# GuanRunwei/Achelous

Hardware: AMD Instinct MI355X
Metric: frames/sec (whole node) EN-GDF-PN-S0 320x320+512pts bs64 @1/2/4/8 GPU (higher is better)
Workload: dtype bf16; 1 GPU; EN-GDF-PN-S0 forward + decode + NMS, 320x320 image + radar map, 512 points, batch 64 per GPU, all 5 heads, seeded random weights; radar_map=256 occupied cells per frame of 102 400 (SURVEY 8d: real maps are > 99 % zeros), global_batch=64, parallelism=batch-sharded x1, launches_per_forward=113

## Files before the change

### achelous_amd/csrc/api.cpp

```cpp
#include <atomic>
#include <cstring>
#include <functional>
#include <string>

#include "engine.h"
#include <map>
#include <mutex>
#include <algorithm>
#include "k_detect.h"
#include "k_prepost.h"
#include "k_train.h"
#include "k_train2.h"
#include "k_train3.h"
#include "k_loss.h"
#include "k_metrics.h"

struct ach_handle {
    ach::EngineBase* eng = nullptr;
    std::string err;
};

static thread_local std::string g_create_error;

template <class F>
// ... 9 lines not shown
        h->err = e.what();
        return ACH_ERR_INVALID;
    } catch (...) {
        h->err = "unknown error";
        return ACH_ERR_INVALID;
    }
}

extern "C" {

int ach_create(const ach_config* cfg, ach_handle** out) {
    if (!cfg || !out) return ACH_ERR_INVALID;
    try {
        if (cfg->backbone != ACH_BACKBONE_EDGENEXT && cfg->backbone != ACH_BACKBONE_MOBILEVIT)
            throw ach::AchError{ACH_ERR_UNSUPPORTED, "backbone must be 'en' or 'mv'"};
        if (cfg->phi < ACH_PHI_S0 || cfg->phi > ACH_PHI_S2) throw ach::AchError{ACH_ERR_UNSUPPORTED, "phi must be S0, S1 or S2"};
        if (cfg->neck != ACH_NECK_GDF && cfg->neck != ACH_NECK_CDF) throw ach::AchError{ACH_ERR_UNSUPPORTED, "neck must be 'gdf' or 'cdf'"};
        if (cfg->pc_seg != ACH_PCSEG_PN && cfg->pc_seg != ACH_PCSEG_PN2 && cfg->pc_seg != ACH_PCSEG_NONE && cfg->pc_seg != ACH_PCSEG_PN2_MSG)
            throw ach::AchError{ACH_ERR_UNSUPPORTED, "pc_seg must be 'pn', 'pn2', 'pn2_msg' or none (Achelous3T)"};
        if (cfg->num_det < 1 || cfg->num_det > 59 || cfg->num_seg < 1 || (cfg->pc_seg != ACH_PCSEG_NONE && (cfg->pc_classes < 1 || cfg->pc_channels < 3)))
            throw ach::AchError{ACH_ERR_INVALID, "bad class / channel counts"};
        ach_handle* h = new ach_handle();
        h->eng = ach::make_engine(*cfg);
        *out = h;
        return ACH_OK;
    } catch (const ach::AchError& e) {
        g_create_error = e.msg;
        return e.code;
    } catch (...) {
        g_create_error = "allocation failure";
        return ACH_ERR_NOMEM;
    }
}

void ach_destroy(ach_handle* h) {
    if (!h) return;
    delete h->eng;
    delete h;
}

const char* ach_last_error(const ach_handle* h) { return h ? h->err.c_str() : g_create_error.c_str(); }

int ach_load_weights(ach_handle* h, const ach_tensor_desc* tensors, size_t n) {
    return guarded(h, [&] { h->eng->load(tensors, n); });
}

int ach_set_option(ach_handle* h, const char* key, int32_t value) {
    return guarded(h, [&] {
        if (!key) throw ach::AchError{ACH_ERR_INVALID, "null option"};
        if (std::string(key) == "full_taps") h->eng->full_taps = value != 0;
        else if (std::string(key) == "streams") h->eng->multi_stream = value != 0;
        else if (std::string(key) == "graph") h->eng->use_graph = value != 0;
        else if (std::string(key) == "fused_mlp") h->eng->fuse_mlp = value != 0;
        else if (std::string(key) == "mlp_split") h->eng->mlp_split = value;
        else if (std::string(key) == "row_conv") h->eng->row_conv = value != 0;
        else if (std::string(key) == "fused_rc") h->eng->fuse_rc = value != 0;
        else if (std::string(key) == "dw_tile") h->eng->dw_tile = value != 0;
        else if (std::string(key) == "stem_mfma") h->eng->stem_mfma = value != 0;
        else if (std::string(key) == "point_stream2") h->eng->point_on_head_stream = value;
        else if (std::string(key) == "head_batch") h->eng->head_batch = value != 0;
        else if (std::string(key) == "head_fuse") h->eng->head_fuse = value != 0;
        else if (std::string(key) == "head_fuse_dbg") h->eng->head_fuse_dbg = value;
        else if (std::string(key) == "side_priority") h->eng->side_low_priority = value;
        else if (std::string(key) == "head_lds_pad") h->eng->head_lds_pad = value < 0 ? 0 : (value > 65536 ? 65536 : value);
        else if (std::string(key) == "head_stream") h->eng->head_stream = value != 0;
        else if (std::string(key) == "split_decoders") h->eng->split_decoders = value;
        else if (std::string(key) == "group_wpc") h->eng->group_wpc = value < 0 ? 0 : value;
        else if (std::string(key) == "group_max") h->eng->group_max = value < 0 ? 0 : value;
        else if (std::string(key) == "dec_fork") h->eng->dec_fork = value < 0 ? 0 : (value > 3 ? 3 : value);
        else if (std::string(key) == "radar_start") h->eng->radar_start = value;
        else if (std::string(key) == "pipeline") h->eng->pipeline = value != 0;
        else if (std::string(key) == "pool_strip") h->eng->pool_strip = value;
        else if (std::string(key) == "fused_mv2") h->eng->fuse_mv2 = value != 0;
        else if (std::string(key) == "dw_even") h->eng->dw_even = value != 0;
        else if (std::string(key) == "xca_mfma") h->eng->xca_mfma = value != 0;
        else if (std::string(key) == "xca_frame") h->eng->xca_frame = value;
        else if (std::string(key) == "xca_fold_mfma") h->eng->xca_fold_mfma = value != 0;
        else if (std::string(key) == "xca_slice") h->eng->xca_slice = value;
        else if (std::string(key) == "xca_front_waves") h->eng->xca_front_waves = value;
        else if (std::string(key) == "xca_back_waves") h->eng->xca_back_waves = value;
        else if (std::string(key) == "gemm_rows") h->eng->gemm_rows = (value == 2 || value == 4) ? value : 1;
        else if (std::string(key) == "radar_rows4") h->eng->radar_rows4 = value;
        else if (std::string(key) == "radar_skip") h->eng->radar_skip = value != 0;
        else if (std::string(key) == "radar_bg") h->eng->radar_bg = value != 0;
        else if (std::string(key) == "radar_pool_sparse") h->eng->radar_pool_sparse = value != 0;
        else if (std::string(key) == "radar_compact") h->eng->radar_compact = value != 0;
        else if (std::string(key) == "head_mfma") h->eng->head_mfma = value != 0;
        else if (std::string(key) == "head_rows") h->eng->head_rows = value;
        else if (std::string(key) == "xwait2_op") h->eng->dbg_xwait2_op = value;
        else if (std::string(key) == "gemm_blocks") h->eng->gemm_blocks = value;
        else if (std::string(key) == "sdta_fuse") h->eng->sdta_fuse = value;
        else if (std::string(key) == "level_chain") h->eng->level_chain = value != 0;
        else if (std::string(key) == "level_rows") h->eng->level_rows = value != 0;
        else if (std::string(key) == "mlp_band") h->eng->mlp_band = value;
        else if (std::string(key) == "mlp_band_run") h->eng->mlp_band_run = value != 0;
        else if (std::string(key) == "mlp_band_dbg") h->eng->mlp_band_dbg = value;
        else if (std::string(key) == "mlp_band_lean") h->eng->mlp_band_lean = value;
        else if (std::string(key) == "head_band") h->eng->head_band = value > 0 ? value : 40;
        else if (std::string(key) == "head_grid") h->eng->head_grid = value;
        else if (std::string(key) == "head_debug") h->eng->head_debug = value;
        else if (std::string(key) == "attn_mfma") h->eng->attn_mfma = value != 0;
        else if (std::string(key) == "ds_fuse") h->eng->ds_fuse = value != 0;
        else if (std::string(key) == "sa_fuse") h->eng->sa_fuse = value != 0;
        else if (std::string(key) == "pn2_fps_all") h->eng->pn2_fps_all = value != 0;
        else if (std::string(key) == "ghost_rb") h->eng->ghost_rb = value > 0 ? value : 5;
        else if (std::string(key) == "pc_chain") h->eng->pc_chain = value != 0;
        else if (std::string(key) == "mlp_split_hw") h->eng->mlp_split_hw = value;
        else if (std::string(key) == "radar_direct") h->eng->radar_direct = value != 0;
        else if (std::string(key) == "mv_stem") h->eng->mv_stem = value != 0;
        else if (std::string(key) == "csp_fuse") h->eng->csp_fuse = value < 0 ? 0 : (value > 2 ? 2 : value);
        else if (std::string(key) == "band_rows_s3") h->eng->band_rows_s3 = value;
        else if (std::string(key) == "spp_split") h->eng->spp_split = value;
        else if (std::string(key) == "ffn_rows2") h->eng->ffn_rows2 = value != 0;
        else if (std::string(key) == "csp_band") h->eng->csp_band = value > 0 ? value : 40;
        else if (std::string(key) == "ghost_fuse") h->eng->ghost_fuse = value != 0;
        else if (std::string(key) == "io_bf16") {
            if (value != 0 && h->eng->cfg.dtype != ACH_DTYPE_F16) throw ach::AchError{ACH_ERR_INVALID, "io_bf16 applies to the fp16-storage engine (ACH_DTYPE_F16) only"};
            h->eng->io_bf16 = value != 0;
        }
        else throw ach::AchError{ACH_ERR_INVALID, std::string("unknown option: ") + key};
    });
}

int ach_plan(ach_handle* h, int32_t batch) {
    return guarded(h, [&] { h->eng->plan(batch); });
}

size_t ach_arena_bytes(const ach_handle* h) { return (h && h->eng) ? h->eng->aarena_used + h->eng->warena_used : 0; }

int ach_forward(ach_handle* h, const void* image, const void* radar, const void* points, void* det3, void* det4, void* det5,
                void* se_seg, void* lane_seg, void* pc_seg, void* stream) {
    return guarded(h, [&] {
        if (h->eng->ops.empty()) throw ach::AchError{ACH_ERR_INVALID, "ach_plan must precede ach_forward"};
        if (!image || !radar || !det3 || !det4 || !det5 || !se_seg || !lane_seg || (h->eng->cfg.pc_seg != ACH_PCSEG_NONE && (!points || !pc_seg)))
            throw ach::AchError{ACH_ERR_INVALID, "null input/output pointer"};
        ach::IoPtrs& io = h->eng->io;
        io.image = image; io.radar = radar; io.points = points;
        io.det[0] = det3; io.det[1] = det4; io.det[2] = det5; io.se = se_seg; io.lane = lane_seg; io.pc = pc_seg;
        h->eng->run(static_cast<hipStream_t>(stream));
        hipError_t e = hipGetLastError();
        if (e != hipSuccess) throw ach::AchError{ACH_ERR_DEVICE, std::string("kernel launch: ") + hipGetErrorString(e)};
    });
}

int ach_forward_detect(ach_handle* h, const void* image, const void* radar, const void* points, void* det3, void* det4, void* det5,
                       void* se_seg, void* lane_seg, void* pc_seg, float* decoded, float conf_thres, float nms_thres, int32_t max_det,
                       float* out_rows, int32_t* out_idx, int32_t* out_count, void* workspace, void* stream) {
    return guarded(h, [&] {
        if (h->eng->ops.empty()) throw ach::AchError{ACH_ERR_INVALID, "ach_plan must precede ach_forward_detect"};
        if (!image || !radar || !det3 || !det4 || !det5 || !se_seg || !lane_seg || (h->eng->cfg.pc_seg != ACH_PCSEG_NONE && (!points || !pc_seg)))
            throw ach::AchError{ACH_ERR_INVALID, "null input/output pointer"};
        if (max_det <= 0 || !decoded || !out_rows || !out_idx || !out_count || !workspace)
            throw ach::AchError{ACH_ERR_INVALID, "bad detect arguments"};
        ach::IoPtrs& io = h->eng->io;
        io.image = image; io.radar = radar; io.points = points;
        io.det[0] = det3; io.det[1] = det4; io.det[2] = det5; io.se = se_seg; io.lane = lane_seg; io.pc = pc_seg;
        ach::EngineBase* e = h->eng;
        const int B = e->batch;
        e->detect_tail = [=](hipStream_t st) {
            e->decode(B, det3, det4, det5, decoded, st);
            e->nms(B, decoded, conf_thres, nms_thres, max_det, out_rows, out_idx, out_count, workspace, st);
        };
        struct Clear { ach::EngineBase* e; ~Clear() { e->detect_tail = nullptr; } } clear{e};
        e->run_eager(static_cast<hipStream_t>(stream));
        hipError_t err = hipGetLastError();
        if (err != hipSuccess) throw ach::AchError{ACH_ERR_DEVICE, std::string("kernel launch: ") + hipGetErrorString(err)};
// ... 644 lines not shown
```

### achelous_amd/csrc/engine.h

```cpp
#pragma once
#include <cstdlib>
#include <cstdio>
#include <functional>
#include <map>
#include <string>
#include <vector>

#include "../../include/achelous.h"
#include "ach_platform.h"

namespace ach {

struct AchError {
    int code;
    std::string msg;
};

struct HostTensor {
    std::vector<float> data;
    std::vector<long> shape;
    long numel() const { long n = 1; for (long s : shape) n *= s; return n; }
};

struct TapInfo {
    const void* ptr = nullptr;
    int kind = 0;
    int B = 0, H = 0, W = 0, C = 0;
    long ld = 0;
    int is_f32 = 0;
    int is_i32 = 0;
    int add_eye = 0;
};

struct Op {
    std::string name;
    std::function<void(hipStream_t)> fn;
    double bytes = 0;
    double layout_bytes = 0;
    double flops = 0;
    int stream = 0;
    int wait_ev = -1, wait_ev2 = -1;
    int signal_ev = -1;
    bool xwait = false;
    bool xsignal = false;
    bool xwait2 = false;
    bool xsignal2 = false;
    bool xwait3 = false;
    bool xsignal3 = false;
};

struct IoPtrs {
    const void* image = nullptr; const void* radar = nullptr; const void* points = nullptr;
    void* det[3] = {nullptr, nullptr, nullptr};
    void* se = nullptr; void* lane = nullptr; void* pc = nullptr;
};

class EngineBase {
public:
    explicit EngineBase(const ach_config& c) : cfg(c) {}
    virtual ~EngineBase();
    ach_config cfg;
    std::map<std::string, HostTensor> weights;
    std::string last_error;

    char* warena = nullptr; size_t warena_cap = 0, warena_used = 0;
    char* aarena = nullptr; size_t aarena_cap = 0, aarena_used = 0;
    bool measuring = false;
    bool use_graph = false;
    bool io_bf16 = false;
    int csp_fuse = 2;
    int band_rows_s3 = 0;
    int spp_split = 0;
    bool ffn_rows2 = true;
    int ffn_rows2_min = 0;
    int csp_band = 40;
    bool ghost_fuse = true;
    bool mv_stem = true;
    bool radar_direct = true;
    bool pc_chain = true;
    int ghost_rb = 5;
    bool pn2_fps_all = true;
    bool sa_fuse = false;
    bool ds_fuse = true;
    bool multi_stream = true;
    int gemm_rows = 1;
    int xca_frame = 0;
    bool xca_fold_mfma = true;
    int xca_slice = 0;
    int xca_front_waves = 0, xca_back_waves = 0;
    bool xca_mfma = true;
    bool dw_even = true;
    int radar_rows4 = 2;
    bool radar_compact = true;
    bool radar_bg = true;
    bool radar_pool_sparse = true;
    bool radar_skip = true;
    int gemm_blocks = 0;
    int sdta_fuse = 1;
    bool level_chain = true;
    int dbg_xwait2_op = -1;
    int head_rows = 2;
    bool level_rows = false;
    int head_band = 40;
    bool head_mfma = false;
    int head_grid = 0;
    int head_debug = 0;
    bool attn_mfma = true;
    bool fuse_mv2 = true;
    bool mlp_band_run = false;
    int mlp_band_lean = 0;
    int mlp_band_dbg = 0;
    int mlp_band = 1;
    bool fuse_mlp = true;
    int group_wpc = 4096;
    int group_max = 1024;
    int dec_fork = 1;
    int split_decoders = 0;
    bool head_stream = false;
    int head_lds_pad = 0;
    int side_low_priority = 3;
    bool pipeline = false;
    int radar_start = -2;
    int radar_start_eff() const { return radar_start == -2 ? ((pipeline && multi_stream) ? 2 : 1) : radar_start; }
    int pool_strip = 2;
    int head_fuse_dbg = 0;
    bool head_fuse = true;
    bool head_batch = true;
    int point_on_head_stream = -1;
    bool stem_mfma = true;
    bool dw_tile = true;
    bool fuse_rc = true;
    bool row_conv = true;
    int mlp_split_hw = 1024;
    int mlp_split = -1;
    bool full_taps = false;
    int batch = 0;
    std::vector<Op> ops;
    std::map<std::string, TapInfo> taps;
    std::vector<std::string> tap_order;
    IoPtrs io;

    void load(const ach_tensor_desc* t, size_t n);
    virtual void plan(int B) = 0;
    void run(hipStream_t s);
    void run_eager(hipStream_t s);
    void join(hipStream_t s);
    long forwards_in_flight() const { return issued - joined; }
    std::function<void(hipStream_t)> detect_tail;
    void run_profiled(hipStream_t s, float* op_ms, size_t cap);
    void set_probe(int op_index) { set_probe_range(0, op_index, op_index); }
    void read_probe(float* avg_ms, int* samples) { read_probe_slot(0, avg_ms, samples); }
    void set_probe_range(int slot, int first, int last);
    void read_probe_slot(int slot, float* avg_ms, int* samples);
    virtual void decode(int B, const void* d3, const void* d4, const void* d5, float* out, hipStream_t s) = 0;
    virtual unsigned long long count_saturated(hipStream_t s) = 0;
    std::vector<std::pair<const void*, size_t>> t_regions;
    void* sat_dev = nullptr; size_t sat_dev_regions = 0;
    void note_region(const void* p, size_t bytes) { if (!measuring) t_regions.emplace_back(p, bytes); }
    void nms(int B, const float* decoded, float conf, float iou, int max_det, float* rows, int* idx, int* count,
             void* workspace, hipStream_t s);
    size_t nms_workspace_bytes(int B) const;
    int num_anchors() const;
    void read_tap(const std::string& name, float* out, size_t cap);
    std::vector<long> tap_shape(const std::string& name) const;
    virtual void preprocess_radar(int B, int C, const float* in, void* out, hipStream_t s) = 0;
    virtual void normalize_points(int B, int N, int D, const float* in, void* out, hipStream_t s) = 0;
    virtual void preprocess_image(int B, const unsigned char* in, void* out, hipStream_t s) = 0;
    virtual void seg_argmax(int B, int C, const void* seg, unsigned char* out, hipStream_t s) = 0;
    virtual void seg_resize_argmax(int B, int C, const void* seg, int out_h, int out_w, float* prob_ws, unsigned char* out, hipStream_t s) = 0;
    void correct_boxes(int B, int max_det, const float* rows, const int* count, int img_h, int img_w, int letterbox, float* out, hipStream_t s);
    float* prepost_scratch = nullptr; size_t prepost_scratch_bytes = 0;
    virtual float bench_gemm(int M, int K, int N, int act, int ln, int residual, int P, int iters, hipStream_t s) = 0;

protected:
    const HostTensor& W(const std::string& key) const;
    bool hasW(const std::string& key) const { return weights.count(key) != 0; }
    void* walloc(size_t bytes);
    void* aalloc(size_t bytes);
// ... 83 lines not shown
```

### achelous_amd/csrc/engine_impl.h

```cpp
#pragma once
#include "engine.h"

#include <algorithm>
#include <cmath>
#include <cstring>

#include "k_dechead.h"
#include "k_csphead.h"
#include "k_upchain.h"
#include "k_detect.h"
#include "k_conv3.h"
#include "k_gemm.h"
#include "k_ghost.h"
#include "k_headdw.h"
#include "k_mlp.h"
#include "k_mlpband.h"
#include "k_mv2.h"
#include "k_mvit.h"
#include "k_nhwc.h"
#include "k_points.h"
#include "k_pn2.h"
#include "k_prepost.h"
#include "k_radar.h"
#include <functional>
#include "k_sdta.h"
#include "k_xca.h"
#include "k_xcaframe.h"

namespace ach {

#define ACH_HIP_CHECK(expr)                                                                               \
    do {                                                                                                  \
        hipError_t e_ = (expr);                                                                           \
        if (e_ != hipSuccess) throw AchError{ACH_ERR_DEVICE, std::string(#expr) + ": " + hipGetErrorString(e_)}; \
    } while (0)

static inline long round_up(long v, long m) { return (v + m - 1) / m * m; }

template <class T>
class Engine final : public EngineBase {
    using S = Store<T>;
    static constexpr int VEC = S::VEC;
    static constexpr int KC = 4 * VEC;
    static constexpr bool H16E = is_h16<T>::value;
    using IOB = typename std::conditional<std::is_same<T, f16_t>::value, bf16_t, T>::type;
    bool io_alt() const { return std::is_same<T, f16_t>::value && io_bf16; }

public:
    explicit Engine(const ach_config& c) : EngineBase(c) {}

    struct A {
        T* p = nullptr; int B = 0, H = 0, W = 0, C = 0; long ld = 0;
        long rows() const { return long(B) * H * W; }
        A slice(int c0, int c) const { A s = *this; s.p = p + c0; s.C = c; return s; }
    };
    struct Pl {
        T* p = nullptr; int B = 0, C = 0, H = 0, W = 0;
    };
    struct Lin { std::vector<float> w, b; int N = 0, K = 0; };

    A alloc(int B, int H, int W, int C) {
        A a; a.B = B; a.H = H; a.W = W; a.C = C; a.ld = round_up(C, 8);
        a.p = static_cast<T*>(aalloc(size_t(a.rows()) * a.ld * sizeof(T)));
        note_region(a.p, size_t(a.rows()) * a.ld * sizeof(T));
        return a;
    }
    A alloc_ld(int B, int H, int W, int C, long ld) {
        A a; a.B = B; a.H = H; a.W = W; a.C = C; a.ld = ld;
        a.p = static_cast<T*>(aalloc(size_t(a.rows()) * a.ld * sizeof(T)));
        note_region(a.p, size_t(a.rows()) * a.ld * sizeof(T));
        return a;
    }
    Pl alloc_pl(int B, int C, int H, int W) {
        Pl a; a.B = B; a.C = C; a.H = H; a.W = W;
        a.p = static_cast<T*>(aalloc(size_t(B) * C * H * W * sizeof(T)));
        note_region(a.p, size_t(B) * C * H * W * sizeof(T));
        return a;
    }
    float* alloc_f32(size_t n) { return static_cast<float*>(aalloc(n * sizeof(float))); }

    T* up_T(const std::vector<float>& v) {
        T* d = static_cast<T*>(walloc(v.size() * sizeof(T)));
        if (!measuring) {
            std::vector<T> h(v.size());
            for (size_t i = 0; i < v.size(); ++i) S::st(&h[i], v[i]);
            ACH_HIP_CHECK(hipMemcpy(d, h.data(), h.size() * sizeof(T), hipMemcpyHostToDevice));
        }
        return d;
    }
    void tap(const std::string& name, const A& a) {
        TapInfo t; t.ptr = a.p; t.kind = 0; t.B = a.B; t.H = a.H; t.W = a.W; t.C = a.C; t.ld = a.ld; add_tap(name, t);
    }
    void tap(const std::string& name, const Pl& a) {
        TapInfo t; t.ptr = a.p; t.kind = 1; t.B = a.B; t.H = a.H; t.W = a.W; t.C = a.C; add_tap(name, t);
// ... 1482 lines not shown

    Lin conv_lin(const std::string& wkey, const std::string& bkey, int Ci, int Cp, int k) const {
        const HostTensor& w = W(wkey);
        const int Co = int(w.shape[0]);
        if (w.numel() != long(Co) * Ci * k * k) throw AchError{ACH_ERR_MISSING_KEY, "conv weight shape: " + wkey};
        Lin l; l.N = Co; l.K = k * k * Cp; l.w.assign(size_t(Co) * l.K, 0.f);
        for (int o = 0; o < Co; ++o)
            for (int c = 0; c < Ci; ++c)
                for (int t = 0; t < k * k; ++t) l.w[size_t(o) * l.K + size_t(t) * Cp + c] = w.data[(size_t(o) * Ci + c) * k * k + t];
        if (!bkey.empty() && hasW(bkey)) l.b = W(bkey).data; else l.b.assign(size_t(Co), 0.f);
        return l;
    }
    A conv_gemm(const std::string& name, const A& x, const Lin& l, int k, int stride, int act, const A* residual = nullptr) {
        const int pad = k / 2;
        const int Ho = (x.H + 2 * pad - k) / stride + 1, Wo = (x.W + 2 * pad - k) / stride + 1;
        A y = alloc(x.B, Ho, Wo, l.N);
        GemmOpt o; o.act = act; o.residual = residual;
        o.conv_k = k; o.conv_s = stride; o.conv_p = pad; o.Hin = x.H; o.Win = x.W; o.Cin = int(x.ld); o.Creal = x.C; o.Ho = Ho; o.Wo = Wo;
        gemm(name, x.p, x.ld, y.rows(), pack(l), y.p, y.ld, o);
        return y;
    }
    struct Bordered { T* p0 = nullptr; T* base = nullptr; int B = 0, H = 0, W = 0, C = 0; long ld = 0, row = 0, img = 0; };
    Bordered alloc_bordered(int B, int H, int W, int C, long ld = 0) {
        Bordered t; t.B = B; t.H = H; t.W = W; t.C = C; t.ld = ld ? ld : round_up(C, 8);
        t.row = long(W + 2) * t.ld; t.img = long(H + 2) * t.row;
        t.base = static_cast<T*>(aalloc(size_t(B) * t.img * sizeof(T)));
        t.p0 = t.base + t.row + t.ld;
        return t;
    }
    A conv3_bordered(const std::string& name, const Bordered& x, const Lin& l, int act, int stride = 1) {
        const int Ho = (x.H - 1) / stride + 1, Wo = (x.W - 1) / stride + 1;
        A y = alloc(x.B, Ho, Wo, l.N);
        const bool half = 2 * x.ld == VEC;
        const int cv = half ? 1 : int(x.ld) / VEC, ks = cdiv(9 * cv, 4);
        Packed pk = pack(l);
        const double bytes = double(x.B) * x.H * x.W * x.C * sizeof(T) + double(y.rows()) * y.C * sizeof(T);
        const double lbytes = double(x.B) * x.H * x.W * x.ld * sizeof(T) + double(y.rows()) * y.ld * sizeof(T);
        const bool shape_ok = (pk.NT == 2 && y.ld == 32 && !half) || (pk.NT == 1 && stride == 2 && y.ld <= 16);
        if (row_conv && shape_ok && (ks == 3 || ks == 5 || ks == 9) && pk.nchunks == 1 && pk.ksteps == ks) {
            std::vector<float> b32(32, 0.f);
            for (int n = 0; n < l.N; ++n) b32[n] = l.b[n];
            Conv3Params cp{x.p0, x.ld, x.row, x.img, y.p, y.ld, pk.w, up_f32(b32), x.B, Ho, Wo, cv, act, 0, nullptr, 0, (radar_rows4 == 2 && Ho % 4 == 0) ? 1 : 0};
            const int NT = pk.NT;
            add_op(name, [cp, ks, NT, stride, half](hipStream_t s) { launch_conv3<T>(cp, ks, NT, stride, s, half); }, bytes, 2.0 * double(y.rows()) * l.K * l.N, lbytes);
            return y;
        }
        if (half) throw AchError{ACH_ERR_INVALID, name + ": 8-byte pixels are only read by the row-walking conv"};
        GemmOpt o; o.act = act;
        o.conv_k = 3; o.conv_s = stride; o.conv_p = 0; o.Hin = x.H + 2; o.Win = x.W + 2; o.Cin = int(x.ld); o.Creal = x.C; o.Ho = Ho; o.Wo = Wo;
        gemm(name, x.base, x.ld, y.rows(), pk, y.p, y.ld, o);
        return y;
    }
    void rcnet(A outs[3]) {
        const int* w = widths();
        const int chans[9] = {3, w[0] / 4, w[0] / 4, w[0] / 4, w[1] / 4, w[1] / 4, w[2] / 4, w[2] / 4, w[3] / 4};
        const bool down[8] = {true, true, false, true, false, true, false, true};
        const int B = batch, R = cfg.resolution;
        const bool narrow0 = fuse_rc && row_conv && chans[0] <= 4 && (R * R) % 4 == 0;
        bool direct0 = false;
        if constexpr (H16E) direct0 = radar_direct && narrow0 && pool_strip > 0 && R % 16 == 0 && R % POOLN_ROWS == 0;
        A x;
        if (direct0) { x.B = B; x.H = R; x.W = R; x.C = 3; x.ld = 4; x.p = nullptr; }
        else x = narrow0 ? alloc_ld(B, R, R, 3, 4) : alloc(B, R, R, 3);
        if (!direct0) {
            ToNhwcParams tp{nullptr, x.p, B, 3, R, R, x.ld};
            const void** rin = &io.radar;
            mark_xwait_next();
            const double bytes = double(x.rows()) * (3 + 3) * sizeof(T), lbytes = double(x.rows()) * (3 + x.ld) * sizeof(T);
            const bool alt = io_alt();
            if (narrow0) {
                const dim3 grid(unsigned(cdivl(x.rows() / 4, 256))), block(256);
                add_op("image_radar_encoder.radar_encoder.to_nhwc", [tp, grid, block, rin, alt](hipStream_t s) mutable { tp.X = *rin; if (alt) ACH_LAUNCH((nchw3_to_nhwc4_kernel<T, IOB>), grid, block, s, tp); else ACH_LAUNCH((nchw3_to_nhwc4_kernel<T, T>), grid, block, s, tp); }, bytes, 0, lbytes);
            } else {
                const dim3 grid(unsigned(cdivl(x.rows(), 256))), block(256);
                add_op("image_radar_encoder.radar_encoder.to_nhwc", [tp, grid, block, rin, alt](hipStream_t s) mutable { tp.X = *rin; if (alt) ACH_LAUNCH((nchw_to_nhwc_kernel<T, IOB>), grid, block, s, tp); else ACH_LAUNCH((nchw_to_nhwc_kernel<T, T>), grid, block, s, tp); }, bytes, 0, lbytes);
            }
        }
        for (int i = 0; i < 8; ++i) {
            const std::string pfx = "image_radar_encoder.radar_encoder.rc_blocks." + std::to_string(i);
            const std::string d = pfx + ".radar_conv.deformable_conv";
            const bool narrow = i == 0 && narrow0;
            const bool half = narrow && 2 * x.ld == VEC;
            const int C = chans[i], Cp = half ? VEC : int(x.ld);
            Bordered pooled = alloc_bordered(B, x.H, x.W, C, narrow ? 4 : 0);
            unsigned short* occ = nullptr;
            int occ_r = 0;
            const bool strip0 = pool_strip > 0 && (C >= 16 || narrow || (pool_strip > 1 && C >= 8));
            if (i == 0 && radar_skip && fuse_rc && strip0 && C <= 4 && x.W % 16 == 0 && x.W / 16 <= 32) {
                const HostTensor& ob = W(d + ".offset_conv.bias");
                float mx = 0.f;
                bool finite = true;
                for (float v : ob.data) { finite = finite && std::isfinite(v); mx = std::max(mx, std::fabs(v)); }
                if (finite && mx <= 13.f) { occ_r = 2 + int(std::floor(mx)); occ = static_cast<unsigned short*>(aalloc(size_t(B) * x.H * (x.W / 16) * sizeof(unsigned short))); }
            }
            if (i == 0 && direct0) {
                if constexpr (H16E) {
                PoolNchwParams pp{nullptr, pooled.p0, pooled.ld, B, x.H, x.W, pooled.row, pooled.img, occ};
                pp.sparse = (radar_pool_sparse && occ) ? 1 : 0;
                const dim3 grid(unsigned(cdivl(long(B) * (x.H / POOLN_ROWS) * (x.W / 4), 256))), block(256);
                const void** rin = &io.radar;
                const bool alt = io_alt();
                mark_xwait_next();
                add_op(pfx + ".avgpool", [pp, grid, block, rin, alt](hipStream_t s) mutable { pp.X = *rin; if (alt) ACH_LAUNCH((avgpool3x3_nchw3_kernel<T, IOB>), grid, block, s, pp); else ACH_LAUNCH((avgpool3x3_nchw3_kernel<T, T>), grid, block, s, pp); },
                       2.0 * x.rows() * C * sizeof(T), 0, double(x.rows()) * (3 + pooled.ld) * sizeof(T));
                }
            } else
            { PoolParams pp{x.p, x.ld, pooled.p0, pooled.ld, B, x.H, x.W, C, pooled.row, pooled.img, occ};
              const double bytes = 2.0 * x.rows() * C * sizeof(T), lbytes = double(x.rows()) * (x.ld + pooled.ld) * sizeof(T);
              const bool strip = pool_strip > 0 && (C >= 16 || narrow || (pool_strip > 1 && C >= 8));
              if (strip) ew(pfx + ".avgpool", avgpool3x3_kernel<T, 4>, pp, long(B) * x.H * cdiv(x.W, 4) * ((C + 3) / 4), bytes, lbytes);
              else ew(pfx + ".avgpool", avgpool3x3_kernel<T, 1>, pp, x.rows() * ((C + 3) / 4), bytes, lbytes); }
            Lin lo = conv_lin(d + ".offset_conv.weight", d + ".offset_conv.bias", C, Cp, 3);
            Lin lm = conv_lin(d + ".modulator_conv.weight", d + ".modulator_conv.bias", C, Cp, 3);
            if (lo.N != 18 || lm.N != 9) throw AchError{ACH_ERR_MISSING_KEY, "deformable conv shapes at " + d};
            Lin lom; lom.N = 27; lom.K = lo.K; lom.w = lo.w; lom.w.insert(lom.w.end(), lm.w.begin(), lm.w.end()); lom.b = lo.b; lom.b.insert(lom.b.end(), lm.b.begin(), lm.b.end());
            const int cvp = half ? 1 : int(pooled.ld) / VEC, ksp = cdiv(9 * cvp, 4);
            const bool fused_front = fuse_rc && C <= 16 && (ksp == 3 || ksp == 5 || ksp == 9);
            A om;
            if (!fused_front) om = conv3_bordered(pfx + ".offmask", pooled, lom, ACT_NONE);
            std::vector<float> sc, sh; bn_coeffs(pfx + ".norm", 1e-5, sc, sh);
            const HostTensor& w1 = W(pfx + ".weight_conv1.weight"); const HostTensor& b1 = W(pfx + ".weight_conv1.bias");
            const HostTensor& w3 = W(d + ".regular_conv.weight");
            if (w3.numel() != long(C) * C * 9 || w1.numel() != long(C) * C) throw AchError{ACH_ERR_MISSING_KEY, "radar block shapes at " + pfx};
            Lin lf; lf.N = C; lf.K = 9 * Cp; lf.w.assign(size_t(C) * lf.K, 0.f); lf.b.assign(size_t(C), 0.f);
            for (int co = 0; co < C; ++co) {
                lf.b[co] = b1.data[co] * sc[co] + sh[co];
                for (int c = 0; c < C; ++c)
                    for (int k = 0; k < 9; ++k) {
                        double acc = 0;
                        for (int m = 0; m < C; ++m) acc += double(w1.data[size_t(co) * C + m]) * sc[co] * w3.data[(size_t(m) * C + c) * 9 + k];
                        lf.w[size_t(co) * lf.K + size_t(k) * Cp + c] = float(acc);
                    }
            }
            A y;
            Bordered yb;
            bool y_bordered = false;
            if (fused_front) {
                Lin lf2 = lf;
                for (float& v : lf2.w) v *= 2.0f;
                Packed pkom = pack(lom), pkf = pack(lf2);
                if (pkom.NT != 2 || pkom.nchunks != 1 || pkom.ksteps != ksp || pkf.NT != 1 || pkf.nchunks != 1 || pkf.ksteps != ksp)
                    throw AchError{ACH_ERR_UNSUPPORTED, "radar block packing at " + pfx};
                std::vector<float> b32(32, 0.f), b16(16, 0.f);
                for (int n = 0; n < 27; ++n) b32[n] = lom.b[n];
                for (int n = 0; n < C; ++n) b16[n] = lf.b[n];
                if (down[i] && row_conv) {
                    yb = alloc_bordered(B, x.H, x.W, C, narrow ? 4 : 0);
                    y_bordered = true;
                } else {
                    y = alloc(B, x.H, x.W, C);
                }
                const long yld = y_bordered ? yb.ld : y.ld;
                RcFrontParams rp{pooled.p0, pooled.ld, pooled.row, pooled.img, pkom.w, up_f32(b32), pkf.w, up_f32(b16), x.p, x.ld,
                                 y_bordered ? yb.p0 : y.p, yld, y_bordered ? yb.row : long(x.W) * y.ld, y_bordered ? yb.img : long(x.H) * x.W * y.ld,
                                 B, x.H, x.W, cvp, C, occ, occ_r, radar_compact ? 1 : 0, (((occ && radar_rows4 == 1) || radar_rows4 == 2) && x.H % 4 == 0) ? 1 : 0, nullptr, 0};
                const bool rdirect = i == 0 && direct0;
                if constexpr (H16E) {
                    if (radar_bg && rdirect && occ && y_bordered && narrow && rp.compact && rp.rows4 && yld <= 4 && x.W <= 512) {
                        rp.prev = static_cast<unsigned short*>(aalloc(size_t(B) * x.H * (x.W / 16) * sizeof(unsigned short)));
                        rp.bg = 1;
                        uint32_t h[4];
                        for (int c = 0; c < 4; ++c) { const float r = c < C ? lf.b[c] : 0.f; h[c] = H16<T>::bits(r > 0.f ? r : 0.f); }
                        FillPx8Params fq{yb.p0, yb.row, yb.img, B, x.H, x.W, make_uint2(h[0] | (h[1] << 16), h[2] | (h[3] << 16))};
                        if (!measuring) post_plan.push_back([fq]() { ACH_LAUNCH(fill_px8_kernel<T>, dim3(unsigned(cdivl(long(fq.B) * fq.H * fq.Wd, 256))), dim3(256), hipStream_t(nullptr), fq); });
                    }
                }
                const void** rres = &io.radar;
                const int rbf = io_alt() ? 1 : 0;
                const double bytes = double(x.rows()) * 3.0 * C * sizeof(T), lbytes = double(x.rows()) * (pooled.ld + x.ld + yld) * sizeof(T);
                add_op(pfx + ".front", [rp, ksp, rdirect, rres, rbf](hipStream_t s) mutable { if (rdirect) { rp.Rn = *rres; rp.rn_bf16 = rbf; } launch_rc_front<T>(rp, ksp, s); }, bytes,
                       2.0 * double(x.rows()) * 9.0 * C * (27 + C), lbytes);
            } else {
            DeformParams dp;
            std::memset(&dp, 0, sizeof(dp));
            dp.pooled = pooled.p0; dp.ldp = pooled.ld; dp.prow = pooled.row; dp.pimg = pooled.img; dp.om = om.p; dp.ldo = om.ld; dp.res = x.p; dp.ldr = x.ld;
            dp.B = B; dp.H = x.H; dp.Wd = x.W; dp.Cp = Cp;
            if (Cp == 8 && (C == 3 || C == 8)) {
                y = alloc(B, x.H, x.W, C);
                dp.Y = y.p; dp.ldy = y.ld; dp.Wf = up_f32(lf.w); dp.bf = up_f32(lf.b);
                const dim3 grid(unsigned(cdivl(x.rows(), 256))), block(256);
                const double bytes = double(x.rows()) * (3.0 * C + 27) * sizeof(T), lbytes = double(x.rows()) * (3.0 * Cp + 32) * sizeof(T);
                if (C == 3) add_op(pfx + ".deform", [dp, grid, block](hipStream_t s) { ACH_LAUNCH((deform_fused_kernel<T, 3, 4>), grid, block, s, dp, dp.Wf, dp.bf); }, bytes, 0, lbytes);
                else add_op(pfx + ".deform", [dp, grid, block](hipStream_t s) { ACH_LAUNCH((deform_fused_kernel<T, 8, 8>), grid, block, s, dp, dp.Wf, dp.bf); }, bytes, 0, lbytes);
            } else {
                A col = alloc(B, x.H, x.W, 9 * Cp);
                dp.Y = col.p; dp.ldy = col.ld;
                ew(pfx + ".deform.sample", deform_sample_kernel<T>, dp, x.rows() * 9 * (Cp / 4), double(x.rows()) * (10.0 * C + 27) * sizeof(T), double(x.rows()) * (10.0 * Cp + 32) * sizeof(T));
                y = alloc(B, x.H, x.W, C);
                GemmOpt o; o.act = ACT_RELU; o.residual = &x;
                gemm(pfx + ".deform.contract", col, pack(lf), y, o);
            }
            }
            const int k = down[i] ? 3 : 1;
            if (y_bordered) x = conv3_bordered(pfx + ".conv2", yb, conv_lin(pfx + ".weight_conv2.weight", pfx + ".weight_conv2.bias", C, half ? VEC : int(yb.ld), 3), ACT_NONE, 2);
            else x = conv_gemm(pfx + ".conv2", y, conv_lin(pfx + ".weight_conv2.weight", pfx + ".weight_conv2.bias", C, int(y.ld), k), k, down[i] ? 2 : 1, ACT_NONE);
            if (x.C != chans[i + 1]) throw AchError{ACH_ERR_MISSING_KEY, "radar width mismatch at " + pfx};
            tap("radar.b" + std::to_string(i), x);
            if (i == 3) outs[0] = x;
            if (i == 5) outs[1] = x;
            if (i == 7) outs[2] = x;
        }
        tap("r3", outs[0]); tap("r4", outs[1]); tap("r5", outs[2]);
    }

    void fuse_all(const A img[3], const A rad[3], A out[3]) {
        const std::string e = "image_radar_encoder";
        Multi6<StatParams> ms; Multi6<EcaParams> me; Multi6<FuseParams> mf;
        std::memset(&ms, 0, sizeof(ms)); std::memset(&me, 0, sizeof(me)); std::memset(&mf, 0, sizeof(mf));
        int n = 0, smax = 1;
        long eca_max = 0, fuse_max = 0;
        double bytes = 0;
        for (int l = 0; l < 3; ++l) {
            const std::string st = std::to_string(3 + l);
            const int Ci = img[l].C, Cr = rad[l].C, HW = img[l].H * img[l].W;
            std::vector<float> sc, sh; bn_coeffs(e + ".norm_stage" + st, 1e-5, sc, sh);
            if (int(sc.size()) != Ci + Cr) throw AchError{ACH_ERR_MISSING_KEY, "fusion norm width"};
            out[l] = alloc(img[l].B, img[l].H, img[l].W, Ci + Cr);
            const A srcs[2] = {img[l], rad[l]};
            int coff = 0;
            for (int h = 0; h < 2; ++h, ++n) {
                const A& x = srcs[h];
                const int S = HW >= 1024 ? 8 : (HW >= 256 ? 4 : 1);
                float* part = alloc_f32(size_t(x.B) * S * 2 * x.C);
                ms.j[n] = StatParams{x.p, x.ld, part, HW, x.C, S};
                smax = std::max(smax, S);
                const HostTensor& wk = W(e + ".channel_attn_stage" + st + "." + std::to_string(h) + ".conv.weight");
                float* scl = alloc_f32(size_t(x.B) * x.C);
                me.j[n] = EcaParams{part, S, up_f32(wk.data), int(wk.numel()), up_f32(std::vector<float>(sc.begin() + coff, sc.begin() + coff + x.C)), scl, x.B, x.C, HW};
// ... 538 lines not shown
```

Baseline: 39730 frames/s.

## Fuse radar block 0 pool, deformable front and strided conv2 into one tiled kernel

```diff
diff --git a/achelous_amd/csrc/api.cpp b/achelous_amd/csrc/api.cpp
--- a/achelous_amd/csrc/api.cpp
+++ b/achelous_amd/csrc/api.cpp
@@ -115,6 +115,8 @@
         else if (std::string(key) == "gemm_rows") h->eng->gemm_rows = (value == 2 || value == 4) ? value : 1;
         else if (std::string(key) == "radar_rows4") h->eng->radar_rows4 = value;
         else if (std::string(key) == "radar_skip") h->eng->radar_skip = value != 0;
+        else if (std::string(key) == "radar_block0") h->eng->radar_block0 = value != 0;
+        else if (std::string(key) == "radar_block0_halo") h->eng->radar_block0_halo = value < 0 ? 0 : (value > 6 ? 6 : value);
         else if (std::string(key) == "radar_bg") h->eng->radar_bg = value != 0;
         else if (std::string(key) == "radar_pool_sparse") h->eng->radar_pool_sparse = value != 0;
         else if (std::string(key) == "radar_compact") h->eng->radar_compact = value != 0;
diff --git a/achelous_amd/csrc/engine.h b/achelous_amd/csrc/engine.h
--- a/achelous_amd/csrc/engine.h
+++ b/achelous_amd/csrc/engine.h
@@ -94,6 +94,8 @@
     bool radar_compact = true;
     bool radar_bg = true;
     bool radar_pool_sparse = true;
+    bool radar_block0 = true;
+    int radar_block0_halo = 3;
     bool radar_skip = true;
     int gemm_blocks = 0;
     int sdta_fuse = 1;
diff --git a/achelous_amd/csrc/engine_impl.h b/achelous_amd/csrc/engine_impl.h
--- a/achelous_amd/csrc/engine_impl.h
+++ b/achelous_amd/csrc/engine_impl.h
@@ -10,6 +10,7 @@
 #include "k_upchain.h"
 #include "k_detect.h"
 #include "k_conv3.h"
+#include "k_rcblock0.h"
 #include "k_gemm.h"
 #include "k_ghost.h"
 #include "k_headdw.h"
@@ -1658,18 +1659,30 @@
             const bool narrow = i == 0 && narrow0;
             const bool half = narrow && 2 * x.ld == VEC;
             const int C = chans[i], Cp = half ? VEC : int(x.ld);
-            Bordered pooled = alloc_bordered(B, x.H, x.W, C, narrow ? 4 : 0);
+            bool block0 = false;
+            int reach0 = 0;
+            if constexpr (H16E) {
+                if (i == 0 && radar_block0 && direct0 && radar_skip && half && down[0] && !full_taps) {
+                    float mx = 0.f;
+                    bool finite = true;
+                    for (float v : W(d + ".offset_conv.bias").data) { finite = finite && std::isfinite(v); mx = std::max(mx, std::fabs(v)); }
+                    if (finite && mx <= float(RB0_HALO - 2)) { reach0 = 2 + int(std::floor(mx)); block0 = true; }
+                }
+            }
+            Bordered pooled;
+            if (!block0) pooled = alloc_bordered(B, x.H, x.W, C, narrow ? 4 : 0);
             unsigned short* occ = nullptr;
             int occ_r = 0;
             const bool strip0 = pool_strip > 0 && (C >= 16 || narrow || (pool_strip > 1 && C >= 8));
-            if (i == 0 && radar_skip && fuse_rc && strip0 && C <= 4 && x.W % 16 == 0 && x.W / 16 <= 32) {
+            if (i == 0 && !block0 && radar_skip && fuse_rc && strip0 && C <= 4 && x.W % 16 == 0 && x.W / 16 <= 32) {
                 const HostTensor& ob = W(d + ".offset_conv.bias");
                 float mx = 0.f;
                 bool finite = true;
                 for (float v : ob.data) { finite = finite && std::isfinite(v); mx = std::max(mx, std::fabs(v)); }
                 if (finite && mx <= 13.f) { occ_r = 2 + int(std::floor(mx)); occ = static_cast<unsigned short*>(aalloc(size_t(B) * x.H * (x.W / 16) * sizeof(unsigned short))); }
             }
-            if (i == 0 && direct0) {
+            if (block0) {
+            } else if (i == 0 && direct0) {
                 if constexpr (H16E) {
                 PoolNchwParams pp{nullptr, pooled.p0, pooled.ld, B, x.H, x.W, pooled.row, pooled.img, occ};
                 pp.sparse = (radar_pool_sparse && occ) ? 1 : 0;
@@ -1720,6 +1733,26 @@
                 std::vector<float> b32(32, 0.f), b16(16, 0.f);
                 for (int n = 0; n < 27; ++n) b32[n] = lom.b[n];
                 for (int n = 0; n < C; ++n) b16[n] = lf.b[n];
+                if constexpr (H16E) if (block0) {
+                    Lin l2 = conv_lin(pfx + ".weight_conv2.weight", pfx + ".weight_conv2.bias", C, VEC, 3);
+                    Packed pk2 = pack(l2);
+                    const int Ho = (x.H - 1) / 2 + 1, Wo = (x.W - 1) / 2 + 1;
+                    A y2 = alloc(B, Ho, Wo, l2.N);
+                    if (pk2.NT != 1 || pk2.nchunks != 1 || pk2.ksteps != 3 || ksp != 3 || y2.ld > 16) throw AchError{ACH_ERR_UNSUPPORTED, "radar block packing at " + pfx};
+                    std::vector<float> b2(32, 0.f);
+                    for (int n = 0; n < l2.N; ++n) b2[n] = l2.b[n];
+                    RcBlock0Params bp{nullptr, io_alt() ? 1 : 0, pkom.w, up_f32(b32), pkf.w, up_f32(b16), pk2.w, up_f32(b2), y2.p, y2.ld, B, x.H, x.W, Ho, Wo,
+                                      reach0, std::max(reach0, radar_block0_halo), cdiv(Wo, RB0_TO), cdiv(Ho, RB0_TO)};
+                    const void** rin = &io.radar;
+                    mark_xwait_next();
+                    const double bytes = double(x.rows()) * 3.0 * sizeof(T) + double(y2.rows()) * y2.C * sizeof(T);
+                    add_op(pfx + ".front+pool+conv2", [bp, rin](hipStream_t s) mutable { bp.X = *rin; launch_rc_block0<T>(bp, s); }, bytes,
+                           2.0 * double(x.rows()) * 9.0 * C * (27 + C) + 2.0 * double(y2.rows()) * l2.K * l2.N, double(x.rows()) * 3.0 * sizeof(T) + double(y2.rows()) * y2.ld * sizeof(T));
+                    x = y2;
+                    if (x.C != chans[i + 1]) throw AchError{ACH_ERR_MISSING_KEY, "radar width mismatch at " + pfx};
+                    tap("radar.b" + std::to_string(i), x);
+                    continue;
+                }
                 if (down[i] && row_conv) {
                     yb = alloc_bordered(B, x.H, x.W, C, narrow ? 4 : 0);
                     y_bordered = true;
diff --git a/achelous_amd/csrc/k_rcblock0.h b/achelous_amd/csrc/k_rcblock0.h
--- /dev/null
+++ b/achelous_amd/csrc/k_rcblock0.h
@@ -0,0 +1,293 @@
+#pragma once
+#include "ach_platform.h"
+#include "k_radar.h"
+#include "k_conv3.h"
+
+namespace ach {
+
+constexpr int RB0_TO = 16;
+constexpr int RB0_YT = 2 * RB0_TO + 1;
+constexpr int RB0_HALO = 6;
+constexpr int RB0_PT = RB0_YT + 2 * RB0_HALO;
+constexpr int RB0_RT = RB0_PT + 2;
+constexpr int RB0_RCH = 7;
+constexpr int RB0_RW = 8 * RB0_RCH;
+
+struct RcBlock0Params {
+    const void* X; int in_bf16;
+    const void* Wom; const float* bom;
+    const void* Wf; const float* bf;
+    const void* W2; const float* b2;
+    void* Y; long ldy;
+    int B, H, Wd, Ho, Wo;
+    int occ_r, halo;
+    int tiles_x, tiles_y;
+};
+
+struct BilinearTapYX { int fy, fx; float w00, w01, w10, w11; };
+__device__ __forceinline__ BilinearTapYX make_tap_yx(float sy, float sx, float mask, int H, int Wd) {
+    BilinearTapYX t;
+    const float cy = clampf(sy, -1.f, float(H)), cx = clampf(sx, -1.f, float(Wd));
+    const float fy = fminf(floorf(cy), float(H - 1)), fx = fminf(floorf(cx), float(Wd - 1));
+    const float ly = cy - fy, lx = cx - fx;
+    const float hym = (1.f - ly) * mask, lym = ly * mask, hx = 1.f - lx;
+    t.w00 = hym * hx; t.w01 = hym * lx; t.w10 = lym * hx; t.w11 = lym * lx;
+    t.fy = int(fy); t.fx = int(fx);
+    return t;
+}
+
+template <class T>
+__global__ __launch_bounds__(256, 2) void rc_block0_kernel(const RcBlock0Params p) { f16_sat_mode<T>();
+    static_assert(sizeof(T) == 2, "16-bit storage");
+    constexpr int KS = 3, YT = RB0_YT, PT = RB0_PT, RW = RB0_RW;
+    __shared__ uint4 rawq[3 * RB0_RT * RB0_RCH];
+    __shared__ uint2 Pl[PT * PT];
+    __shared__ uint2 yl[YT * YT];
+    __shared__ float oml[4][16][36];
+    __shared__ uint4 wsh[KS * 3 * 64];
+    __shared__ unsigned char fl[PT * PT + 7];
+    __shared__ unsigned long long hm[PT], am[YT];
+    __shared__ unsigned short plist[YT * YT + 7];
+    __shared__ int ntot_s;
+    const uint16_t* rawl = reinterpret_cast<const uint16_t*>(rawq);
+
+    const int tid = threadIdx.x, lane = tid & 63, wave = wave_uniform(tid >> 6);
+    const int px = lane & 15, g = lane >> 4;
+    const unsigned wg = xcd_block(blockIdx.x, gridDim.x);
+    const unsigned per_img = unsigned(p.tiles_x) * unsigned(p.tiles_y);
+    const int b = int(wg / per_img), trem = int(wg - unsigned(b) * per_img);
+    const int tyi = trem / p.tiles_x, txi = trem - tyi * p.tiles_x;
+    const int oy0 = tyi * RB0_TO, ox0 = txi * RB0_TO;
+    const int h = p.halo, PTr = YT + 2 * h, RTr = PTr + 2;
+    const int yy0 = 2 * oy0 - 1, yx0 = 2 * ox0 - 1;
+    const int py0 = yy0 - h, px0 = yx0 - h;
+    const int ry0 = py0 - 1, rx0 = px0 - 1;
+    const int ax0 = rx0 & ~7;
+    const int nch = ((rx0 + RTr - 1) >> 3) - (ax0 >> 3) + 1;
+    const long cstride = long(p.H) * p.Wd;
+    const uint16_t* Xb = static_cast<const uint16_t*>(p.X) + long(b) * 3 * cstride;
+    auto recast = [&](uint32_t w) { return p.in_bf16 ? h16_recast<bf16_t, T>(w) : w; };
+    auto val = [](uint32_t bits) { return H16<T>::lo(bits & 0xffffu); };
+
+    for (int i = tid; i < KS * 3 * 64; i += 256) {
+        const int f = i >> 6, l = i & 63;
+        wsh[i] = f < 2 * KS ? static_cast<const uint4*>(p.Wom)[f * 64 + l] : static_cast<const uint4*>(p.Wf)[(f - 2 * KS) * 64 + l];
+    }
+    {
+        const bool al16 = (reinterpret_cast<uintptr_t>(p.X) & 15u) == 0;
+        const int per_plane = RTr * nch;
+        for (int i = tid; i < 3 * per_plane; i += 256) {
+            const int c = i / per_plane, rem = i - c * per_plane;
+            const int r = rem / nch, k = rem - r * nch;
+            const int gy = ry0 + r, gx = ax0 + 8 * k;
+            const bool in = gy >= 0 && gy < p.H && gx >= 0 && gx + 8 <= p.Wd;
+            const uint16_t* src = Xb + c * cstride + (in ? long(gy) * p.Wd + gx : 0);
+            uint4 v;
+            if (al16) v = *reinterpret_cast<const uint4*>(src);
+            else { const uint2 a = *reinterpret_cast<const uint2*>(src), bq = *reinterpret_cast<const uint2*>(src + 4); v = make_uint4(a.x, a.y, bq.x, bq.y); }
+            v = make_uint4(in ? recast(v.x) : 0u, in ? recast(v.y) : 0u, in ? recast(v.z) : 0u, in ? recast(v.w) : 0u);
+            rawq[(c * RB0_RT + r) * RB0_RCH + k] = v;
+        }
+    }
+    __syncthreads();
+    auto raw_at = [&](int c, int gy, int gx) -> uint32_t { return rawl[(c * RB0_RT + (gy - ry0)) * RW + (gx - ax0)]; };
+    for (int i = tid; i < PTr * PTr; i += 256) {
+        const int r = i / PTr, c = i - r * PTr;
+        const int gy = py0 + r, gx = px0 + c;
+        const bool in = gy >= 0 && gy < p.H && gx >= 0 && gx < p.Wd;
+        float acc[4];
+        int nz = 0;
+        ACH_UNROLL
+        for (int ch = 0; ch < 3; ++ch) {
+            float col[3];
+            ACH_UNROLL
+            for (int j = 0; j < 3; ++j) {
+                const float up = val(raw_at(ch, gy - 1, gx - 1 + j)), mid = val(raw_at(ch, gy, gx - 1 + j)), dn = val(raw_at(ch, gy + 1, gx - 1 + j));
+                col[j] = ((0.f + up) + mid) + dn;
+                if (j == 1) nz |= !(mid == 0.f) ? 1 : 0;
+            }
+            acc[ch] = ((col[0] + col[1]) + col[2]) * (1.0f / 9.0f);
+            nz |= !(acc[ch] == 0.f) ? 1 : 0;
+        }
+        acc[3] = 0.f;
+        Pl[r * PT + c] = in ? make_uint2(H16<T>::pack(acc[0], acc[1]), H16<T>::pack(acc[2], acc[3])) : make_uint2(0u, 0u);
+        fl[r * PT + c] = static_cast<unsigned char>(in ? nz : 0);
+    }
+    __syncthreads();
+    if (tid < PTr) {
+        unsigned long long m = 0;
+        for (int c = 0; c < PTr; ++c) m |= (unsigned long long)(fl[tid * PT + c]) << c;
+        unsigned long long d = m;
+        for (int k = 1; k <= p.occ_r; ++k) d |= (m << k) | (m >> k);
+        hm[tid] = d;
+    }
+    __syncthreads();
+    if (tid < YT) {
+        unsigned long long a = 0;
+        for (int dr = -p.occ_r; dr <= p.occ_r; ++dr) a |= hm[tid + h + dr];
+        a = (a >> h) & ((1ull << YT) - 1ull);
+        const int gy = yy0 + tid;
+        if (gy < 0 || gy >= p.H) a = 0;
+        if (yx0 < 0) a &= ~((1ull << (-yx0)) - 1ull);
+        const int lim = p.Wd - yx0;
+        if (lim < YT) a &= lim > 0 ? ((1ull << lim) - 1ull) : 0ull;
+        am[tid] = a;
+    }
+    __syncthreads();
+    if (tid < YT) {
+        int base = 0;
+        for (int q = 0; q < tid; ++q) base += __popcll(am[q]);
+        unsigned long long m = am[tid];
+        if (tid == YT - 1) ntot_s = base + __popcll(m);
+        for (; m; m &= m - 1ull) plist[base++] = static_cast<unsigned short>((tid << 6) | (__ffsll(static_cast<long long>(m)) - 1));
+    }
+    {
+        float b0[4];
+        ACH_UNROLL
+        for (int i = 0; i < 4; ++i) b0[i] = p.bf[i];
+        for (int i = tid; i < YT * YT; i += 256) {
+            const int yr = i / YT, xc = i - yr * YT;
+            const int gy = yy0 + yr, gx = yx0 + xc;
+            if (gy < 0 || gy >= p.H || gx < 0 || gx >= p.Wd) { yl[i] = make_uint2(0u, 0u); continue; }
+            if ((am[yr] >> xc) & 1ull) continue;
+            float ov[4];
+            ACH_UNROLL
+            for (int c = 0; c < 4; ++c) { const float rr = c < 3 ? val(raw_at(c < 3 ? c : 0, gy, gx)) : 0.f; const float r = 0.f + b0[c]; ov[c] = (r > 0.f ? r : 0.f) + rr; }
+            yl[i] = make_uint2(H16<T>::pack(ov[0], ov[1]), H16<T>::pack(ov[2], ov[3]));
+        }
+    }
+    __syncthreads();
+    {
+        float bv[8], bo[4];
+        ACH_UNROLL
+        for (int i = 0; i < 8; ++i) bv[i] = p.bom[g * 8 + i];
+        ACH_UNROLL
+        for (int i = 0; i < 4; ++i) bo[i] = p.bf[g * 4 + i];
+        auto graw = [&](int c, int y, int x) -> float {
+            const bool in = y >= 0 && y < p.H && x >= 0 && x < p.Wd;
+            const uint32_t bits = Xb[c * cstride + (in ? long(y) * p.Wd + x : 0)];
+            const float v = val(recast(bits));
+            return in ? v : 0.f;
+        };
+        auto pooled_far = [&](int y, int x) -> uint2 {
+            if (y < 0 || y >= p.H || x < 0 || x >= p.Wd) return make_uint2(0u, 0u);
+            float acc[4];
+            ACH_UNROLL
+            for (int ch = 0; ch < 3; ++ch) {
+                float col[3];
+                ACH_UNROLL
+                for (int j = 0; j < 3; ++j) col[j] = ((0.f + graw(ch, y - 1, x - 1 + j)) + graw(ch, y, x - 1 + j)) + graw(ch, y + 1, x - 1 + j);
+                acc[ch] = ((col[0] + col[1]) + col[2]) * (1.0f / 9.0f);
+            }
+            acc[3] = 0.f;
+            return make_uint2(H16<T>::pack(acc[0], acc[1]), H16<T>::pack(acc[2], acc[3]));
+        };
+        auto unpack4 = [](const uint2& v, float (&o)[4]) { o[0] = H16<T>::lo(v.x); o[1] = H16<T>::hi(v.x); o[2] = H16<T>::lo(v.y); o[3] = H16<T>::hi(v.y); };
+        const int ntot = ntot_s;
+        const int ctiles = (ntot + 15) / 16;
+        for (int tile = wave; tile < ctiles; tile += 4) {
+            const int idx = tile * 16 + px;
+            const bool valid = idx < ntot;
+            const int e = plist[valid ? idx : ntot - 1];
+            const int yr = e >> 6, xc = e & 63;
+            const int gy = yy0 + yr, gx = yx0 + xc;
+            const uint2* Pc = Pl + (yr + h) * PT + (xc + h);
+            {
+                f32x4 a0, a1;
+                a0[0] = a0[1] = a0[2] = a0[3] = 0.f;
+                a1[0] = a1[1] = a1[2] = a1[3] = 0.f;
+                ACH_UNROLL
+                for (int s = 0; s < KS; ++s) {
+                    const int tap = 4 * s + g, ty = tap / 3, tx = tap - 3 * ty;
+                    const uint2 v = Pc[tap < 9 ? (ty - 1) * PT + (tx - 1) : 0];
+                    const uint4 xf = make_uint4(v.x, v.y, 0u, 0u);
+                    mfma16<T>(wsh[(s * 2) * 64 + lane], xf, a0);
+                    mfma16<T>(wsh[(s * 2 + 1) * 64 + lane], xf, a1);
+                }
+                float* o = &oml[wave][px][g * 8];
+                *reinterpret_cast<float4*>(o) = make_float4(a0[0] + bv[0], a0[1] + bv[1], a0[2] + bv[2], a0[3] + bv[3]);
+                *reinterpret_cast<float4*>(o + 4) = make_float4(a1[0] + bv[4], a1[1] + bv[5], a1[2] + bv[6], a1[3] + bv[7]);
+            }
+            wave_sync();
+            f32x4 acc;
+            acc[0] = acc[1] = acc[2] = acc[3] = 0.f;
+            ACH_UNROLL
+            for (int s = 0; s < KS; ++s) {
+                const int q = 4 * s + g, ty = q / 3, tx = q - 3 * ty;
+                const bool livetap = q < 9;
+                const int tap = livetap ? q : 0;
+                const float* om = &oml[wave][px][0];
+                const float dy = om[2 * tap], dx = om[2 * tap + 1], ml = om[18 + tap];
+                const float ybase = float(gy + ty - 1), xbase = float(tx - 1);
+                const BilinearTapYX t = make_tap_yx(ybase + dy, float(gx) + xbase + dx, sigmoid_mod(ml), p.H, p.Wd);
+                const float live = livetap ? 1.f : 0.f;
+                const float w00 = t.w00 * live, w01 = t.w01 * live, w10 = t.w10 * live, w11 = t.w11 * live;
+                const int ly = t.fy - py0, lx = t.fx - px0;
+                uint2 A, Bq, Cq, D;
+                if (ly >= 0 && ly + 1 < PTr && lx >= 0 && lx + 1 < PTr) {
+                    const uint2* c0 = Pl + ly * PT + lx;
+                    A = c0[0]; Bq = c0[1]; Cq = c0[PT]; D = c0[PT + 1];
+                } else {
+                    A = pooled_far(t.fy, t.fx); Bq = pooled_far(t.fy, t.fx + 1); Cq = pooled_far(t.fy + 1, t.fx); D = pooled_far(t.fy + 1, t.fx + 1);
+                }
+#if !defined(ACH_HOSTEMU) && ACH_RCF_PK16
+                if constexpr (std::is_same<T, f16_t>::value) {
+                    float q00 = w00, q01 = w01, q10 = w10, q11 = w11;
+                    asm volatile("" : "+v"(q00), "+v"(q01), "+v"(q10), "+v"(q11));
+                    const rcf_h2 h00 = {_Float16(q00), _Float16(q00)}, h01 = {_Float16(q01), _Float16(q01)}, h10 = {_Float16(q10), _Float16(q10)}, h11 = {_Float16(q11), _Float16(q11)};
+                    const uint4 fr = make_uint4(rcf_blend_h2(A.x, Bq.x, Cq.x, D.x, h00, h01, h10, h11), rcf_blend_h2(A.y, Bq.y, Cq.y, D.y, h00, h01, h10, h11), 0u, 0u);
+                    mfma16<T>(wsh[(2 * KS + s) * 64 + lane], fr, acc);
+                    continue;
+                }
+#endif
+                float v[8], a[4], bq[4], cc[4], d[4];
+                unpack4(A, a); unpack4(Bq, bq); unpack4(Cq, cc); unpack4(D, d);
+                ACH_UNROLL
+                for (int i = 0; i < 4; ++i) { v[i] = w00 * a[i] + w01 * bq[i] + w10 * cc[i] + w11 * d[i]; v[4 + i] = 0.f; }
+                mfma16<T>(wsh[(2 * KS + s) * 64 + lane], frag_pack<T>(v), acc);
+            }
+            wave_sync();
+            if (valid && g == 0) {
+                float ov[4];
+                ACH_UNROLL
+                for (int i = 0; i < 4; ++i) { const float rr = i < 3 ? val(raw_at(i < 3 ? i : 0, gy, gx)) : 0.f; const float r = acc[i] + bo[i]; ov[i] = (r > 0.f ? r : 0.f) + rr; }
+                yl[yr * YT + xc] = make_uint2(H16<T>::pack(ov[0], ov[1]), H16<T>::pack(ov[2], ov[3]));
+            }
+        }
+    }
+    __syncthreads();
+    {
+        uint4 wf[KS];
+        ACH_UNROLL
+        for (int s = 0; s < KS; ++s) wf[s] = static_cast<const uint4*>(p.W2)[s * 64 + lane];
+        float bv[4];
+        ACH_UNROLL
+        for (int i = 0; i < 4; ++i) bv[i] = p.b2[g * 4 + i];
+        for (int r = wave; r < RB0_TO; r += 4) {
+            const int oy = oy0 + r, ox = ox0 + px;
+            const uint2* yc = yl + (2 * r + 1) * YT + (2 * px + 1);
+            f32x4 acc;
+            acc[0] = acc[1] = acc[2] = acc[3] = 0.f;
+            ACH_UNROLL
+            for (int s = 0; s < KS; ++s) {
+                const int tap = 4 * s + g, ty = tap / 3, tx = tap - 3 * ty;
+                const uint2 v = yc[tap < 9 ? (ty - 1) * YT + (tx - 1) : 0];
+                mfma16<T>(wf[s], make_uint4(v.x, v.y, 0u, 0u), acc);
+            }
+            if (oy < p.Ho && ox < p.Wo && g * 4 < int(p.ldy)) {
+                float o[4];
+                ACH_UNROLL
+                for (int i = 0; i < 4; ++i) o[i] = acc[i] + bv[i];
+                Store<T>::st4(static_cast<T*>(p.Y) + ((long(b) * p.Ho + oy) * p.Wo + ox) * p.ldy + g * 4, o);
+            }
+        }
+    }
+}
+
+template <class T>
+inline void launch_rc_block0(const RcBlock0Params& p, hipStream_t stream) {
+    const dim3 grid(unsigned(p.B) * unsigned(p.tiles_x) * unsigned(p.tiles_y)), block(256);
+    ACH_LAUNCH((rc_block0_kernel<T>), grid, block, stream, p);
+}
+
+}
```

New measurement: 36270 frames/s. 0.913x the previous value.
